# 2025-comprehensive-design/AudioLDM-with-LoRA

Hardware: AMD Instinct MI355X
Metric: unet_denoise_steps_per_sec (higher is better)
Workload: dtype bf16; 1 GPU; audioldm-s-full-v2 UNet + rank-4 LoRA (q,k,v,out), DDIM 200-step schedule, batch 4 x 10 s clips (latent 250x16), CFG 2.5 (UNet batch 8), bf16; per_gpu_batch=4, parallelism=prompt-sharded x1, hip_graph=True, graph_chains=1

## Files before the change

### audioldm_with_lora_amd/csrc/igemm_halo.hip

```cpp
#include "igemm_core.h"
#include "gn_stats.h"

namespace aldm_igemm_detail {

template <int BM, int BN, int WM, int WN, int HP , int S, int EPI , bool GNIN = false>
__global__ __launch_bounds__(512) void igemm_halo_kernel(const IgemmDev p) {
#if defined(__HIP_DEVICE_COMPILE__)
  aldm_touch_kernargs<sizeof(IgemmDev)>();
  static_assert(WM * WN == 8, "8 waves");
  constexpr int NT = 512, RPP = NT / 8;
  constexpr int MI = BM / WM / 16, NI = BN / WN / 16;
  constexpr int W_PASSES = BN / RPP;
  constexpr int D = S - 1;
  constexpr bool STAGGER = false;
  constexpr int HALO_BYTES = HP * RPP * 128;
  constexpr int BSTAGE = BN * 128;
  constexpr unsigned OOB = 0x80000000u;
  static_assert(BN % RPP == 0, "weight tile rows must be whole DMA passes");
  static_assert((D - 1) * W_PASSES + HP < 64, "vmcnt immediate");

  extern __shared__ __attribute__((aligned(16))) char smem[];
  char* const Hs = smem;
  char* const Bring = smem + 2 * HALO_BYTES;
  float* const gtab = reinterpret_cast<float*>(smem + 2 * HALO_BYTES + S * BSTAGE);

  const int tid = threadIdx.x, lane = tid & 63;
  const int wave = __builtin_amdgcn_readfirstlane(tid >> 6);
  const int wm = wave / WN, wn = wave % WN;
  const int W = p.OW, H = p.OH;
  const int HW2 = W + 2;
  const int rows_pt = BM / W;
  const int tpi = (H + rows_pt - 1) / rows_pt;
  int wid = blockIdx.x, split = 0;
  if constexpr (EPI == 3) {
    split = fdiv(wid, p.fd_tiles_m);
    wid -= split * p.tiles_m;
  }
  const int tile_m = fdiv(wid, p.fd_tiles_n), tile_n = wid - tile_m * p.tiles_n;
  const int img = tile_m / tpi, ty0 = (tile_m - img * tpi) * rows_pt;
  const int m0 = img * p.OHW + ty0 * W, n0 = tile_n * BN;
  const int halo_rows = (rows_pt + 2) * HW2;

  const __amdgpu_buffer_rsrc_t rs_x = make_rsrc(p.x, p.x_bytes);
  const __amdgpu_buffer_rsrc_t rs_x2 = make_rsrc(p.x2 ? (const void*)p.x2 : (const void*)p.x, p.x2 ? p.x2_bytes : p.x_bytes);
  const __amdgpu_buffer_rsrc_t rs_w = make_rsrc(p.w, p.w_bytes);

  const int rbase = tid >> 3;
  const int kchunk = (tid & 7) ^ ((rbase >> 1) & 7);
  int h_pix[HP];
  {
    const FastDiv fd_w2 = {p.fd_halo.mul, p.fd_halo.shift};
    const bool up = p.UH > 0;
#pragma unroll
    for (int ps = 0; ps < HP; ++ps) {
      const int hp = rbase + RPP * ps;
      const int hy = fdiv(hp, fd_w2), hx = hp - hy * HW2;
      const int gy = ty0 - 1 + hy, gx = hx - 1;
      const bool ok = hp < halo_rows && (unsigned)gy < (unsigned)H && (unsigned)gx < (unsigned)W;
      const int sy = !up ? gy : (p.UH == 2 * p.IH ? (gy >> 1) : (gy * p.IH) / p.UH);
      const int sx = !up ? gx : (p.UW == 2 * p.IW ? (gx >> 1) : (gx * p.IW) / p.UW);
      h_pix[ps] = ok ? (img * p.IH + sy) * p.IW + sx : -1;
    }
  }
  unsigned b_off[W_PASSES];
#pragma unroll
  for (int ps = 0; ps < W_PASSES; ++ps) {
    const int row = min(n0 + rbase + RPP * ps, p.N - 1);
    b_off[ps] = (unsigned)row * (unsigned)p.Kpad * 2u + kchunk * 16;
  }

  const int nchunks = p.Ctot >> 6;
  const int c_begin = EPI == 3 ? split * (p.kt_per_split / 9) : 0;
  const int c_end = EPI == 3 ? min(nchunks, c_begin + p.kt_per_split / 9) : nchunks;
  const int nitems = (c_end - c_begin) * 9;
  int i_c = c_begin, i_tap = 0;
  auto issue = [&](int item, int stage) {
    const bool live = item < nitems;
    char* bdst = Bring + stage * BSTAGE + wave * 1024;
    if (live && i_tap == 0) {
      const int c0 = i_c << 6;
      const bool src2 = c0 >= p.Cin;
      const int Cs = src2 ? p.Cin2 : p.Cin;
      const int soff = (c0 - (src2 ? p.Cin : 0)) * 2;
      char* hdst = Hs + (i_c & 1) * HALO_BYTES + wave * 1024;
#pragma unroll
      for (int ps = 0; ps < HP; ++ps) {
        const unsigned off = h_pix[ps] >= 0 ? (unsigned)h_pix[ps] * (unsigned)(Cs * 2) + kchunk * 16 : OOB;
        if (src2) __builtin_amdgcn_raw_ptr_buffer_load_lds(rs_x2, (lds_ptr_t)(hdst + ps * (RPP * 128)), 16, off, soff, 0, 0);
        else __builtin_amdgcn_raw_ptr_buffer_load_lds(rs_x, (lds_ptr_t)(hdst + ps * (RPP * 128)), 16, off, soff, 0, 0);
      }
    }
    const int ksoff = live ? (i_tap * p.Ctot + (i_c << 6)) * 2 : 0;
#pragma unroll
    for (int ps = 0; ps < W_PASSES; ++ps)
      __builtin_amdgcn_raw_ptr_buffer_load_lds(rs_w, (lds_ptr_t)(bdst + ps * (RPP * 128)), 16, live ? b_off[ps] : OOB, ksoff, 0, 0);
    if (live) {
      if (++i_tap == 9) { i_tap = 0; ++i_c; }
    }
  };

  f32x4 acc[MI][NI];
#pragma unroll
  for (int i = 0; i < MI; ++i)
#pragma unroll
    for (int j = 0; j < NI; ++j) acc[i][j] = f32x4{0.f, 0.f, 0.f, 0.f};

  const int lrow = lane & 15, lq = lane >> 4;
  int a_hp[MI];
  {
    const FastDiv fd_w = p.fd_ow;
#pragma unroll
    for (int i = 0; i < MI; ++i) {
      const int pl = wm * (BM / WM) + i * 16 + lrow;
      const int ly = fdiv(pl, fd_w), lx = pl - ly * W;
      a_hp[i] = ly * HW2 + lx;
    }
  }

  auto mma_tap = [&](const char* As, const char* Bs, int tap_off) {
#pragma unroll
    for (int ks = 0; ks < 2; ++ks) {
      const int ch = ks * 4 + lq;
      bf16x8 af[MI], wf[NI];
#pragma unroll
      for (int i = 0; i < MI; ++i) {
        const int r = a_hp[i] + tap_off;
        af[i] = *reinterpret_cast<const bf16x8*>(As + r * 128 + swz(r, ch) * 16);
      }
#pragma unroll
      for (int j = 0; j < NI; ++j) {
        const int r = wn * (BN / WN) + j * 16 + lrow;
        wf[j] = *reinterpret_cast<const bf16x8*>(Bs + r * 128 + swz(r, ch) * 16);
      }
#pragma unroll
      for (int i = 0; i < MI; ++i)
#pragma unroll
        for (int j = 0; j < NI; ++j)
          acc[i][j] = __builtin_amdgcn_mfma_f32_16x16x32_bf16(wf[j], af[i], acc[i][j], 0, 0, 0);
    }
  };

#pragma unroll
  for (int s = 0; s < D; ++s) issue(s, s);
  if constexpr (GNIN) {
    const float my_gamma = tid < p.Ctot ? p.gi_gamma[tid] : 0.f, my_beta = tid < p.Ctot ? p.gi_beta[tid] : 0.f;
    const int groups = p.gi_groups, Cg = p.Ctot / groups;
    int lpg = 1;
    while (lpg * 2 * groups <= NT && lpg < 64) lpg *= 2;
    const GnSrc s1{p.x, p.gi_q1, p.Cin, p.gi_bm1, p.gi_tpi1}, s2{p.x2, p.gi_q2, p.Cin2, p.gi_bm2 > 0 ? p.gi_bm2 : 1, p.gi_tpi2};
    const int HWs = p.IH * p.IW;
    const int g = tid / lpg, j = tid - g * lpg;
    float a = 0.f, q2 = 0.f;
    if (g < groups) gn_group_sums(s1, s2, img, HWs, Cg, g, j, lpg, a, q2);
    for (int o = 1; o < lpg; o <<= 1) { a += __shfl_xor(a, o, 64); q2 += __shfl_xor(q2, o, 64); }
    if (g < groups && j == 0) {
      const float n = (float)HWs * (float)Cg;
      const float mu = a / n;
      gtab[1024 + g] = mu;
      gtab[1088 + g] = rsqrtf(fmaxf(q2 / n - mu * mu, 0.f) + p.gi_eps);
    }
    __syncthreads();
    if (tid < p.Ctot) {
      const int gg = tid / Cg;
      const float sc = my_gamma * gtab[1088 + gg];
      gtab[tid] = sc;
      gtab[512 + tid] = my_beta - gtab[1024 + gg] * sc;
    }
    __syncthreads();
  }
  {
    int st = 0, st_fill = D;
    int c_c = c_begin, c_tap = 0, c_dy = 0, c_dx = 0;
    for (int item = 0; item < nitems; ++item) {
      bool halo_young = false;
#pragma unroll
      for (int d = 1; d < D; ++d) {
        const int t = c_tap + d;
        halo_young = halo_young || ((t == 9 || t == 18) && item + d < nitems);
      }
      if (halo_young) wait_vmcnt<(D - 1) * W_PASSES + HP>(); else wait_vmcnt<(D - 1) * W_PASSES>();
      if constexpr (GNIN) {
        if (c_tap == 0) {
          const int cb = (c_c << 6) + kchunk * 8;
          const f32x4 sc0 = *reinterpret_cast<const f32x4*>(gtab + cb), sc1 = *reinterpret_cast<const f32x4*>(gtab + cb + 4);
          const f32x4 sh0 = *reinterpret_cast<const f32x4*>(gtab + 512 + cb), sh1 = *reinterpret_cast<const f32x4*>(gtab + 512 + cb + 4);
          char* hb = Hs + (c_c & 1) * HALO_BYTES + wave * 1024 + lane * 16;
#pragma unroll
          for (int ps = 0; ps < HP; ++ps) {
            if (h_pix[ps] >= 0) {
              const bf16x8 v = *reinterpret_cast<const bf16x8*>(hb + ps * (RPP * 128));
              bf16x8 o;
#pragma unroll
              for (int k = 0; k < 8; ++k) {
                float t = fmaf((float)v[k], k < 4 ? sc0[k & 3] : sc1[k & 3], k < 4 ? sh0[k & 3] : sh1[k & 3]);
                if (p.gi_act == ALDM_ACT_SILU) t = silu_f(t);
                o[k] = (bf16)t;
              }
              *reinterpret_cast<bf16x8*>(hb + ps * (RPP * 128)) = o;
            }
          }
          __builtin_amdgcn_s_waitcnt(0xC07F);
        }
      }
      __builtin_amdgcn_s_barrier();
      if (!(STAGGER && wave >= 4)) issue(item + D, st_fill);
      mma_tap(Hs + (c_c & 1) * HALO_BYTES, Bring + st * BSTAGE, c_dy * HW2 + c_dx);
      if (STAGGER && wave >= 4) issue(item + D, st_fill);
      st = (st + 1 == S) ? 0 : st + 1;
      st_fill = (st_fill + 1 == S) ? 0 : st_fill + 1;
      ++c_tap;
      if (++c_dx == 3) { c_dx = 0; ++c_dy; }
      if (c_tap == 9) { c_tap = 0; c_dy = 0; ++c_c; }
    }
  }
  wait_vmcnt<0>();
  __builtin_amdgcn_s_barrier();

  IgemmDev q = p;
  q.M = min(p.M, min(m0 + BM, (img + 1) * p.OHW));
  q.qtile = tile_m;
  igemm_epilogue<BM, BN, MI, NI, false, NT, EPI>(q, acc, smem, false, m0, n0, wm * (BM / WM), wn * (BN / WN), lrow, lq, split, tid, nullptr);
#endif
}

template <int BM, int BN, int WM, int WN, int HP, int S, int EPI, bool GNIN = false, bool EXT = false>
__global__ __launch_bounds__(768) void igemm_halo_ws_kernel(const IgemmDev p) {
#if defined(__HIP_DEVICE_COMPILE__)
  aldm_touch_kernargs<sizeof(IgemmDev)>();
  static_assert(WM * WN == 8, "8 compute waves");
  constexpr int NTC = 512, NTL = 256, RPP = NTL / 8;
  constexpr int MI = BM / WM / 16, NI = BN / WN / 16;
  constexpr int HPL = HP * 64 / RPP;
  constexpr int W_PASSES = BN / RPP;
  constexpr int D = S - 1;
  constexpr int HALO_BYTES = HP * 64 * 128;
  constexpr int BSTAGE = BN * 128;
  constexpr unsigned OOB = 0x80000000u;
  static_assert((D - 1) * (W_PASSES + HPL) < 64, "vmcnt immediate");
  static_assert(!EXT || (S == 3 && !GNIN), "fused-shortcut form: ring 3, no gnin_*");
  constexpr int NB = EXT ? 3 : 2;

  extern __shared__ __attribute__((aligned(16))) char smem[];
  char* const Hs = smem;
  char* const Bring = smem + NB * HALO_BYTES;
  float* const gtab = reinterpret_cast<float*>(smem + NB * HALO_BYTES + S * BSTAGE);

  const int tid = threadIdx.x, lane = tid & 63;
  const int wave = __builtin_amdgcn_readfirstlane(tid >> 6);
  const bool loader = wave >= NTC / 64;
  const int W = p.OW, H = p.OH;
  const int KWt = p.KW, NTAP = p.KH * p.KW;
  const int HW2 = W + (p.KW - 1) * p.dw;
  const int rows_pt = BM / W;
  const int tpi = (H + rows_pt - 1) / rows_pt;
  int wid = blockIdx.x, split = 0;
  if constexpr (EPI == 3) {
    split = fdiv(wid, p.fd_tiles_m);
    wid -= split * p.tiles_m;
  }
  const int tile_m = fdiv(wid, p.fd_tiles_n), tile_n = wid - tile_m * p.tiles_n;
  const int img = tile_m / tpi, ty0 = (tile_m - img * tpi) * rows_pt;
  const int m0 = img * p.OHW + ty0 * W, n0 = tile_n * BN;
  const int halo_rows = (rows_pt + (p.KH - 1) * p.dh) * HW2;
  const int nchunks = p.Ctot >> 6;
  const int cps = EPI == 3 ? fdiv(p.kt_per_split, p.fd_kw) : 0;
  const int c_begin = EPI == 3 ? split * cps : 0;
  const int c_end = EPI == 3 ? min(nchunks, c_begin + cps) : nchunks;
  const int next = EXT ? (p.C3tot >> 6) : 0;
  const int eps = EPI == 3 ? (next + p.splits - 1) / p.splits : next;
  const int e_begin = EPI == 3 ? min(next, split * eps) : 0;
  const int e_end = min(next, e_begin + eps);
  const int nmain = (c_end - c_begin) * NTAP;
  const int nitems = nmain + (e_end - e_begin);

  if constexpr (GNIN) {
    float my_gamma = 0.f, my_beta = 0.f;
    if (tid < p.Ctot) { my_gamma = p.gi_gamma[tid]; my_beta = p.gi_beta[tid]; }
    const int groups = p.gi_groups, Cg = p.Ctot / groups;
    if (tid < NTC) {
      int lpg = 1;
      while (lpg * 2 * groups <= NTC && lpg < 64) lpg *= 2;
      const GnSrc s1{p.x, p.gi_q1, p.Cin, p.gi_bm1, p.gi_tpi1}, s2{p.x2, p.gi_q2, p.Cin2, p.gi_bm2 > 0 ? p.gi_bm2 : 1, p.gi_tpi2};
      const int HWs = p.IH * p.IW;
      const int g = tid / lpg, j = tid - g * lpg;
      float a = 0.f, q2 = 0.f;
      if (g < groups) gn_group_sums(s1, s2, img, HWs, Cg, g, j, lpg, a, q2);
      for (int o = 1; o < lpg; o <<= 1) { a += __shfl_xor(a, o, 64); q2 += __shfl_xor(q2, o, 64); }
      if (g < groups && j == 0) {
        const float n = (float)HWs * (float)Cg;
        const float mu = a / n;
        gtab[1024 + g] = mu;
        gtab[1088 + g] = rsqrtf(fmaxf(q2 / n - mu * mu, 0.f) + p.gi_eps);
      }
    }
    __syncthreads();
    if (tid < p.Ctot) {
      const int gg = tid / Cg;
      const float sc = my_gamma * gtab[1088 + gg];
      gtab[tid] = sc;
      gtab[512 + tid] = my_beta - gtab[1024 + gg] * sc;
    }
    __syncthreads();
  }

  if (loader) {
    const int lt = tid - NTC, lwave = wave - NTC / 64;
    const __amdgpu_buffer_rsrc_t rs_x = make_rsrc(p.x, p.x_bytes);
    const __amdgpu_buffer_rsrc_t rs_x2 = make_rsrc(p.x2 ? (const void*)p.x2 : (const void*)p.x, p.x2 ? p.x2_bytes : p.x_bytes);
    const __amdgpu_buffer_rsrc_t rs_w = make_rsrc(p.w, p.w_bytes);
    const int rbase = lt >> 3;
    const int kchunk = (lt & 7) ^ ((rbase >> 1) & 7);
    int h_pix[HPL];
    {
      const FastDiv fd_w2 = {p.fd_halo.mul, p.fd_halo.shift};
      const bool up = p.UH > 0;
#pragma unroll
      for (int ps = 0; ps < HPL; ++ps) {
        const int hp = rbase + RPP * ps;
        const int hy = fdiv(hp, fd_w2), hx = hp - hy * HW2;
        const int gy = ty0 - p.ph + hy, gx = hx - p.pw;
        const bool ok = hp < halo_rows && (unsigned)gy < (unsigned)H && (unsigned)gx < (unsigned)W;
      const int sy = !up ? gy : (p.UH == 2 * p.IH ? (gy >> 1) : (gy * p.IH) / p.UH);
      const int sx = !up ? gx : (p.UW == 2 * p.IW ? (gx >> 1) : (gx * p.IW) / p.UW);
        h_pix[ps] = ok ? (img * p.IH + sy) * p.IW + sx : -1;
      }
    }
    unsigned b_off[W_PASSES];
#pragma unroll
    for (int ps = 0; ps < W_PASSES; ++ps) {
      const int row = min(n0 + rbase + RPP * ps, p.N - 1);
      b_off[ps] = (unsigned)row * (unsigned)p.Kpad * 2u + kchunk * 16;
    }
    int i_c = c_begin, i_tap = 0, i_u = 0;
    bool i_ext = EXT && nmain == 0;
    if (i_ext) i_c = e_begin;
    auto issue = [&](int item, int stage) {
      const bool live = item < nitems;
      char* bdst = Bring + stage * BSTAGE + lwave * 1024;
      if (live && i_tap == 0) {
        const int c0 = i_c << 6;
        char* hdst = Hs + (EXT ? i_u % 3 : (i_c & 1)) * HALO_BYTES + lwave * 1024;
        if (EXT && i_ext) {
          const bool s4 = c0 >= p.Cin3;
          const int Cs = s4 ? p.Cin4 : p.Cin3;
          const int soff = (c0 - (s4 ? p.Cin3 : 0)) * 2;
          const __amdgpu_buffer_rsrc_t rs_e = s4 ? make_rsrc(p.x4, p.x4_bytes) : make_rsrc(p.x3, p.x3_bytes);
#pragma unroll
          for (int ps = 0; ps < HPL; ++ps) {
            const unsigned off = h_pix[ps] >= 0 ? (unsigned)h_pix[ps] * (unsigned)(Cs * 2) + kchunk * 16 : OOB;
            __builtin_amdgcn_raw_ptr_buffer_load_lds(rs_e, (lds_ptr_t)(hdst + ps * (RPP * 128)), 16, off, soff, 0, 0);
          }
        } else {
          const bool src2 = c0 >= p.Cin;
          const int Cs = src2 ? p.Cin2 : p.Cin;
          const int soff = (c0 - (src2 ? p.Cin : 0)) * 2;
#pragma unroll
          for (int ps = 0; ps < HPL; ++ps) {
            const unsigned off = h_pix[ps] >= 0 ? (unsigned)h_pix[ps] * (unsigned)(Cs * 2) + kchunk * 16 : OOB;
            if (src2) __builtin_amdgcn_raw_ptr_buffer_load_lds(rs_x2, (lds_ptr_t)(hdst + ps * (RPP * 128)), 16, off, soff, 0, 0);
            else __builtin_amdgcn_raw_ptr_buffer_load_lds(rs_x, (lds_ptr_t)(hdst + ps * (RPP * 128)), 16, off, soff, 0, 0);
          }
        }
      }
      const int ksoff = !live ? 0 : (EXT && i_ext) ? (NTAP * p.Ctot + (i_c << 6)) * 2 : (i_tap * p.Ctot + (i_c << 6)) * 2;
#pragma unroll
      for (int ps = 0; ps < W_PASSES; ++ps)
        __builtin_amdgcn_raw_ptr_buffer_load_lds(rs_w, (lds_ptr_t)(bdst + ps * (RPP * 128)), 16, live ? b_off[ps] : OOB, ksoff, 0, 0);
      if (live) {
        if (EXT && i_ext) { ++i_c; ++i_u; }
        else if (++i_tap == NTAP) {
          i_tap = 0; ++i_c; ++i_u;
          if (EXT && i_c == c_end) { i_ext = true; i_c = e_begin; }
        }
      }
    };
#pragma unroll
    for (int s = 0; s < D; ++s) issue(s, s);
    int st_fill = D;
    int c_c = c_begin, c_tap = 0;
    for (int item = 0; item < nitems; ++item) {
      int young = 0;
#pragma unroll
      for (int d = 1; d < D; ++d) {
        const int t = c_tap + d, it = item + d;
        const bool opens = it < nitems && (it >= nmain || (it < nmain && (t == NTAP || t == 2 * NTAP)));
        young += opens ? 1 : 0;
      }
      if (young == 0) wait_vmcnt<(D - 1) * W_PASSES>();
      else if (young == 1 || D < 3) wait_vmcnt<(D - 1) * W_PASSES + HPL>();
      else wait_vmcnt<(D - 1) * W_PASSES + (D > 2 ? 2 : 1) * HPL>();
      if constexpr (GNIN) {
        if (c_tap == 0) {
          const int cb = (c_c << 6) + kchunk * 8;
          const f32x4 sc0 = *reinterpret_cast<const f32x4*>(gtab + cb), sc1 = *reinterpret_cast<const f32x4*>(gtab + cb + 4);
          const f32x4 sh0 = *reinterpret_cast<const f32x4*>(gtab + 512 + cb), sh1 = *reinterpret_cast<const f32x4*>(gtab + 512 + cb + 4);
          char* hb = Hs + (c_c & 1) * HALO_BYTES + lwave * 1024 + lane * 16;
#pragma unroll
          for (int ps = 0; ps < HPL; ++ps) {
            if (h_pix[ps] >= 0) {
              const bf16x8 v = *reinterpret_cast<const bf16x8*>(hb + ps * (RPP * 128));
              bf16x8 o;
#pragma unroll
              for (int k = 0; k < 8; ++k) {
                float t = fmaf((float)v[k], k < 4 ? sc0[k & 3] : sc1[k & 3], k < 4 ? sh0[k & 3] : sh1[k & 3]);
                if (p.gi_act == ALDM_ACT_SILU) t = silu_f(t);
                o[k] = (bf16)t;
              }
              *reinterpret_cast<bf16x8*>(hb + ps * (RPP * 128)) = o;
            }
          }
          __builtin_amdgcn_s_waitcnt(0xC07F);
        }
      }
      __builtin_amdgcn_s_barrier();
      issue(item + D, st_fill);
      st_fill = (st_fill + 1 == S) ? 0 : st_fill + 1;
      if (item < nmain && ++c_tap == NTAP) { c_tap = 0; ++c_c; }
    }
    wait_vmcnt<0>();
    __builtin_amdgcn_s_barrier();
    return;
  }

  const int wm = wave / WN, wn = wave % WN;
  f32x4 acc[MI][NI];
#pragma unroll
  for (int i = 0; i < MI; ++i)
#pragma unroll
    for (int j = 0; j < NI; ++j) acc[i][j] = f32x4{0.f, 0.f, 0.f, 0.f};
  const int lrow = lane & 15, lq = lane >> 4;
  int a_hp[MI];
#pragma unroll
  for (int i = 0; i < MI; ++i) {
    const int pl = wm * (BM / WM) + i * 16 + lrow;
    const int ly = fdiv(pl, p.fd_ow), lx = pl - ly * W;
    a_hp[i] = ly * HW2 + lx;
  }
  {
    int st = 0, c_c = c_begin, c_tap = 0, c_dy = 0, c_dx = 0, c_u = 0;
    for (int item = 0; item < nitems; ++item) {
      __builtin_amdgcn_s_barrier();
      const bool seg = EXT && item >= nmain;
      const char* As = Hs + (EXT ? c_u % 3 : (c_c & 1)) * HALO_BYTES;
      const char* Bs = Bring + st * BSTAGE;
      const int tap_off = seg ? HW2 + 1 : c_dy * p.dh * HW2 + c_dx * p.dw;
#pragma unroll
      for (int ks = 0; ks < 2; ++ks) {
        const int ch = ks * 4 + lq;
        bf16x8 af[MI], wf[NI];
#pragma unroll
        for (int i = 0; i < MI; ++i) {
          const int r = a_hp[i] + tap_off;
          af[i] = *reinterpret_cast<const bf16x8*>(As + r * 128 + swz(r, ch) * 16);
        }
#pragma unroll
        for (int j = 0; j < NI; ++j) {
          const int r = wn * (BN / WN) + j * 16 + lrow;
          wf[j] = *reinterpret_cast<const bf16x8*>(Bs + r * 128 + swz(r, ch) * 16);
        }
#pragma unroll
        for (int i = 0; i < MI; ++i)
#pragma unroll
          for (int j = 0; j < NI; ++j) acc[i][j] = __builtin_amdgcn_mfma_f32_16x16x32_bf16(wf[j], af[i], acc[i][j], 0, 0, 0);
      }
      st = (st + 1 == S) ? 0 : st + 1;
      if (seg) { ++c_u; continue; }
      ++c_tap;
      if (++c_dx == KWt) { c_dx = 0; ++c_dy; }
      if (c_tap == NTAP) { c_tap = 0; c_dy = 0; ++c_c; ++c_u; }
    }
  }
  __builtin_amdgcn_s_waitcnt(0xC07F);
  __builtin_amdgcn_s_barrier();
  IgemmDev q = p;
  q.M = min(p.M, min(m0 + BM, (img + 1) * p.OHW));
  q.qtile = tile_m;
  igemm_epilogue<BM, BN, MI, NI, false, NTC, EPI>(q, acc, smem, false, m0, n0, wm * (BM / WM), wn * (BN / WN), lrow, lq, split, tid, nullptr);
#endif
}

template <int BM, int BN, int WM, int WN, int HP, int S, int EPI, bool GNIN = false, bool WS = false, bool EXT = false>
int launch_halo_v(const IgemmDev& d, hipStream_t st) {
  static_assert(!EXT || WS, "the fused-shortcut form exists for the wave-specialised kernel only");
  constexpr size_t lds_loop = (EXT ? 3 : 2) * (size_t)HP * 64 * 128 + (size_t)S * BN * 128 + (GNIN ? (1024 + 128) * sizeof(float) : 0);
  constexpr size_t lds = lds_loop > (size_t)EpiCfg<BM, BN>::BYTES ? lds_loop : (size_t)EpiCfg<BM, BN>::BYTES;
  static_assert(lds <= 160 * 1024, "LDS budget");
  static unsigned long long attr_done = 0;
  void (*kern)(const IgemmDev);
  if constexpr (EXT) kern = igemm_halo_ws_kernel<BM, BN, WM, WN, HP, S, EPI, false, true>;
  else if constexpr (WS) kern = igemm_halo_ws_kernel<BM, BN, WM, WN, HP, S, EPI, GNIN>;
  else kern = igemm_halo_kernel<BM, BN, WM, WN, HP, S, EPI, GNIN>;
  if (int rc = aldm_set_max_lds(reinterpret_cast<const void*>(kern), (int)lds, &attr_done, "igemm_halo")) return rc;
  const int rows_pt = BM / d.OW;
  const int need = WS ? (rows_pt + (d.KH - 1) * d.dh) * (d.OW + (d.KW - 1) * d.dw) : (rows_pt + 2) * (d.OW + 2);
  if (BM % d.OW != 0 || need > HP * 64) {
    aldm_set_error("igemm_halo: image width %d / filter %dx%d does not fit the %dx%d halo tile (%d halo rows of %d)", d.OW, d.KH, d.KW, BM, BN, need, HP * 64);
    return ALDM_E_UNSUPPORTED;
  }
  IgemmDev dd = d;
  if (WS) dd.fd_kw = make_fastdiv((unsigned)(d.KH * d.KW));
  dd.tiles_n = cdiv(d.N, BN);
  dd.fd_tiles_n = make_fastdiv((unsigned)dd.tiles_n);
  dd.fd_halo = make_fastdiv((unsigned)(WS ? d.OW + (d.KW - 1) * d.dw : d.OW + 2));
  const int tpi = cdiv(d.OH, rows_pt);
  dd.tiles_m = d.B * tpi * dd.tiles_n;
  dd.fd_tiles_m = make_fastdiv((unsigned)dd.tiles_m);
  dim3 grid(d.B * tpi * dd.tiles_n * (EPI == 3 ? d.splits : 1), 1, 1);
  hipLaunchKernelGGL(kern, grid, dim3(WS ? 768 : 512), lds, st, dd);
  return aldm_launch_status("igemm_halo");
}

template <int BM, int BN, int WM, int WN, int HP, int S>
int launch_halo_ext(const IgemmDev& d, hipStream_t st) {
  if (d.gi_gamma) {
    aldm_set_error("igemm_halo: gnin_* launches take no second-source segment");
    return ALDM_E_UNSUPPORTED;
  }
  if (d.splits > 1) return launch_halo_v<BM, BN, WM, WN, HP, S, 3, false, true, true>(d, st);
  if (d.out_act == ALDM_ACT_NONE && d.post_act == ALDM_ACT_NONE)
    return d.qstat ? launch_halo_v<BM, BN, WM, WN, HP, S, 4, false, true, true>(d, st) : launch_halo_v<BM, BN, WM, WN, HP, S, 1, false, true, true>(d, st);
  return launch_halo_v<BM, BN, WM, WN, HP, S, 0, false, true, true>(d, st);
}

template <int BM, int BN, int WM, int WN, int HP, int S, bool WS = false>
int launch_halo(const IgemmDev& d, hipStream_t st) {
  if (d.splits > 1) {
    if (d.gi_gamma) {
      aldm_set_error("igemm_halo: gnin_* launches are not split");
      return ALDM_E_UNSUPPORTED;
    }
    return launch_halo_v<BM, BN, WM, WN, HP, S, 3, false, WS>(d, st);
  }
  if (d.gi_gamma) {
    if (d.out_act != ALDM_ACT_NONE || d.post_act != ALDM_ACT_NONE) {
      aldm_set_error("igemm_halo: gnin_* launches take no output activation");
      return ALDM_E_UNSUPPORTED;
    }
    return d.qstat ? launch_halo_v<BM, BN, WM, WN, HP, S, 4, true, WS>(d, st) : launch_halo_v<BM, BN, WM, WN, HP, S, 1, true, WS>(d, st);
  }
  if (d.out_act == ALDM_ACT_NONE && d.post_act == ALDM_ACT_NONE)
    return d.qstat ? launch_halo_v<BM, BN, WM, WN, HP, S, 4, false, WS>(d, st) : launch_halo_v<BM, BN, WM, WN, HP, S, 1, false, WS>(d, st);
  return launch_halo_v<BM, BN, WM, WN, HP, S, 0, false, WS>(d, st);
}

}

int aldm_launch_halo(const aldm_igemm_detail::IgemmDev& d0, int tile, int ring, hipStream_t st) {
  using namespace aldm_igemm_detail;
  IgemmDev d = d0;
  const bool ws = tile == ALDM_TILE_HALO_128x128_WS || tile == ALDM_TILE_HALO_64x128_WS;
  if (ws && d.KH == 1 && d.OH == 1 && d.IH == 1 && d.UH == 0 && d.ph == 0 && d.dh == 1 && d.sh == 1 && d.C3tot == 0 && !d.gi_gamma) {
    d.KH = d.KW; d.KW = 1; d.dh = d.dw; d.dw = 1; d.ph = d.pw; d.pw = 0;
    d.OH = d.OW; d.OW = 1; d.IH = d.IW; d.IW = 1; d.sh = d.sw; d.sw = 1;
    d.fd_ow = make_fastdiv(1u);
    d.fd_ohw = make_fastdiv((unsigned)d.OHW);
  }
  const bool same = ws ? (d.KH % 2 == 1 && d.KW % 2 == 1 && 2 * d.ph == (d.KH - 1) * d.dh && 2 * d.pw == (d.KW - 1) * d.dw &&
                          ((d.KH == 3 && d.KW == 3 && d.dh == 1 && d.dw == 1) || (d.C3tot == 0 && !d.gi_gamma && d.UH == 0)))
                       : (d.KH == 3 && d.KW == 3 && d.ph == 1 && d.pw == 1 && d.dh == 1 && d.dw == 1);
  const bool ok = same && d.sh == 1 && d.sw == 1 &&
                  d.in_act == ALDM_ACT_NONE && d.Cin % 64 == 0 && d.Cin2 % 64 == 0 && d.dilate == 0 &&
                  !d.ln_s && !d.geglu && d.x_bytes < 0x80000000u && d.x2_bytes < 0x80000000u &&
                  ((d.UH == 0 && d.UW == 0) || (d.UH > 0 && d.UW > 0)) && d.OH == (d.UH ? d.UH : d.IH) && d.OW == (d.UW ? d.UW : d.IW);
  if (!ok) {
    aldm_set_error("igemm_halo: needs a stride-1 'same' convolution on the LDS-DMA path (Cin %% 64 == 0, no gather activation): 3x3, or -- wave-specialised tiles -- any odd filter with dilation");
    return ALDM_E_UNSUPPORTED;
  }
  if (d.C3tot > 0) {
    const bool fits = d.UH == 0 && d.C3tot % 64 == 0 && d.Cin3 % 64 == 0 && d.x3_bytes < 0x80000000u && d.x4_bytes < 0x80000000u;
    if (fits && tile == ALDM_TILE_HALO_128x128_WS && (128 / d.OW + 2) * (d.OW + 2) <= 192) return launch_halo_ext<128, 128, 4, 2, 3, 3>(d, st);
    if (fits && tile == ALDM_TILE_HALO_64x128_WS) return launch_halo_ext<64, 128, 2, 4, 2, 3>(d, st);
    aldm_set_error("igemm_halo: the second-source segment needs a wave-specialised halo tile whose halo fits three DMA passes (OW >= 8 at 128 rows)");
    return ALDM_E_UNSUPPORTED;
  }
  if (tile == ALDM_TILE_HALO_128x128_WS) {
    if ((128 / d.OW + (d.KH - 1) * d.dh) * (d.OW + (d.KW - 1) * d.dw) > 192) {
      if (ring == 4) return launch_halo<128, 128, 4, 2, 5, 4, true>(d, st);
      return launch_halo<128, 128, 4, 2, 5, 3, true>(d, st);
    }
    if (ring == 4) return launch_halo<128, 128, 4, 2, 3, 4, true>(d, st);
    return launch_halo<128, 128, 4, 2, 3, 3, true>(d, st);
  }
  if (tile == ALDM_TILE_HALO_64x128_WS) {
    if (ring == 4) return launch_halo<64, 128, 2, 4, 2, 4, true>(d, st);
    return launch_halo<64, 128, 2, 4, 2, 3, true>(d, st);
  }
  if (tile == ALDM_TILE_HALO_128x128) {
    if ((128 / d.OW + 2) * (d.OW + 2) > 192) {
      if (ring == 2) return launch_halo<128, 128, 4, 2, 5, 2>(d, st);
      if (ring == 4) return launch_halo<128, 128, 4, 2, 5, 4>(d, st);
      return launch_halo<128, 128, 4, 2, 5, 3>(d, st);
    }
    if (ring == 2) return launch_halo<128, 128, 4, 2, 3, 2>(d, st);
    if (ring == 4) return launch_halo<128, 128, 4, 2, 3, 4>(d, st);
    return launch_halo<128, 128, 4, 2, 3, 3>(d, st);
  }
  if (ring == 2) return launch_halo<64, 128, 2, 4, 2, 2>(d, st);
  if (ring == 4) return launch_halo<64, 128, 2, 4, 2, 4>(d, st);
  return launch_halo<64, 128, 2, 4, 2, 3>(d, st);
}
```

Baseline: 356.9 denoise_steps/s.

## Overlap GroupNorm stats with ring prefill and share halo normalisation across waves

For the wave-specialised GroupNorm-fused conv kernel, two new forms are added and both are on by default through environment switches. Ring-first lets the loader waves issue the initial weight and halo DMA before the compute waves finish the GroupNorm statistics and tables, so the stats prologue overlaps the first loads. Shared normalisation spreads the in-LDS normalise+SiLU of each halo chunk across all 768 threads, with extra barriers, instead of leaving it to the loader waves alone. The cost is added barrier synchronisation per channel chunk and more template instantiations.

```diff
diff --git a/audioldm_with_lora_amd/csrc/igemm_halo.hip b/audioldm_with_lora_amd/csrc/igemm_halo.hip
--- a/audioldm_with_lora_amd/csrc/igemm_halo.hip
+++ b/audioldm_with_lora_amd/csrc/igemm_halo.hip
@@ -1,3 +1,5 @@
+#include <cstdlib>
+
 #include "igemm_core.h"
 #include "gn_stats.h"
 
@@ -223,7 +225,7 @@
 #endif
 }
 
-template <int BM, int BN, int WM, int WN, int HP, int S, int EPI, bool GNIN = false, bool EXT = false>
+template <int BM, int BN, int WM, int WN, int HP, int S, int EPI, bool GNIN = false, bool EXT = false, bool RF = false, bool SH = false>
 __global__ __launch_bounds__(768) void igemm_halo_ws_kernel(const IgemmDev p) {
 #if defined(__HIP_DEVICE_COMPILE__)
   aldm_touch_kernargs<sizeof(IgemmDev)>();
@@ -238,6 +240,10 @@
   constexpr unsigned OOB = 0x80000000u;
   static_assert((D - 1) * (W_PASSES + HPL) < 64, "vmcnt immediate");
   static_assert(!EXT || (S == 3 && !GNIN), "fused-shortcut form: ring 3, no gnin_*");
+  static_assert(GNIN || (!RF && !SH), "ring-first / shared normalisation are forms of the gnin_* launches");
+  constexpr int NT = NTC + NTL;
+  constexpr int NPP = (HP * 512 + NT - 1) / NT;
+  static_assert(((NT / 8) >> 1) % 8 == 0, "a thread's pieces share one XOR term, hence one channel base");
   constexpr int NB = EXT ? 3 : 2;
 
   extern __shared__ __attribute__((aligned(16))) char smem[];
@@ -273,7 +279,7 @@
   const int nmain = (c_end - c_begin) * NTAP;
   const int nitems = nmain + (e_end - e_begin);
 
-  if constexpr (GNIN) {
+  auto gn_tables = [&]() __attribute__((always_inline)) {
     float my_gamma = 0.f, my_beta = 0.f;
     if (tid < p.Ctot) { my_gamma = p.gi_gamma[tid]; my_beta = p.gi_beta[tid]; }
     const int groups = p.gi_groups, Cg = p.Ctot / groups;
@@ -301,7 +307,50 @@
       gtab[512 + tid] = my_beta - gtab[1024 + gg] * sc;
     }
     __syncthreads();
-  }
+  };
+  if constexpr (GNIN && !RF) gn_tables();
+
+  int sh_cb = 0;
+  unsigned sh_ok = 0;
+  auto sh_setup = [&]() __attribute__((always_inline)) {
+    const FastDiv fd_w2 = {p.fd_halo.mul, p.fd_halo.shift};
+    const int r0 = tid >> 3;
+    sh_cb = ((tid & 7) ^ ((r0 >> 1) & 7)) * 8;
+#pragma unroll
+    for (int k = 0; k < NPP; ++k) {
+      const int hp = r0 + (NT / 8) * k;
+      const int hy = fdiv(hp, fd_w2), hx = hp - hy * HW2;
+      const int gy = ty0 - p.ph + hy, gx = hx - p.pw;
+      const bool ok = hp < HP * 64 && hp < halo_rows && (unsigned)gy < (unsigned)H && (unsigned)gx < (unsigned)W;
+      sh_ok |= ok ? 1u << k : 0u;
+    }
+  };
+  auto sh_norm = [&](int c) __attribute__((always_inline)) {
+    if (sh_ok) {
+      const int cb = (c << 6) + sh_cb;
+      const f32x4 sc0 = *reinterpret_cast<const f32x4*>(gtab + cb), sc1 = *reinterpret_cast<const f32x4*>(gtab + cb + 4);
+      const f32x4 sh0 = *reinterpret_cast<const f32x4*>(gtab + 512 + cb), sh1 = *reinterpret_cast<const f32x4*>(gtab + 512 + cb + 4);
+      char* hb = Hs + (c & 1) * HALO_BYTES + tid * 16;
+      bf16x8 v[NPP];
+#pragma unroll
+      for (int k = 0; k < NPP; ++k)
+        if ((k + 1) * NT <= HP * 512 || tid + k * NT < HP * 512) v[k] = *reinterpret_cast<const bf16x8*>(hb + k * (NT * 16));
+#pragma unroll
+      for (int k = 0; k < NPP; ++k) {
+        if ((sh_ok >> k) & 1u) {
+          bf16x8 o;
+#pragma unroll
+          for (int e = 0; e < 8; ++e) {
+            float t = fmaf((float)v[k][e], e < 4 ? sc0[e & 3] : sc1[e & 3], e < 4 ? sh0[e & 3] : sh1[e & 3]);
+            if (p.gi_act == ALDM_ACT_SILU) t = silu_f(t);
+            o[e] = (bf16)t;
+          }
+          *reinterpret_cast<bf16x8*>(hb + k * (NT * 16)) = o;
+        }
+      }
+    }
+    __builtin_amdgcn_s_waitcnt(0xC07F);
+  };
 
   if (loader) {
     const int lt = tid - NTC, lwave = wave - NTC / 64;
@@ -376,6 +425,11 @@
     };
 #pragma unroll
     for (int s = 0; s < D; ++s) issue(s, s);
+    if constexpr (SH) sh_setup();
+    if constexpr (RF) {
+      __builtin_amdgcn_s_barrier();
+      __builtin_amdgcn_s_barrier();
+    }
     int st_fill = D;
     int c_c = c_begin, c_tap = 0;
     for (int item = 0; item < nitems; ++item) {
@@ -389,7 +443,21 @@
       if (young == 0) wait_vmcnt<(D - 1) * W_PASSES>();
       else if (young == 1 || D < 3) wait_vmcnt<(D - 1) * W_PASSES + HPL>();
       else wait_vmcnt<(D - 1) * W_PASSES + (D > 2 ? 2 : 1) * HPL>();
-      if constexpr (GNIN) {
+      if constexpr (SH) {
+        if (c_tap == 0) {
+          __builtin_amdgcn_s_barrier();
+          issue(item + D, st_fill);
+          sh_norm(c_c);
+          __builtin_amdgcn_s_barrier();
+        } else {
+          __builtin_amdgcn_s_barrier();
+          issue(item + D, st_fill);
+        }
+        st_fill = (st_fill + 1 == S) ? 0 : st_fill + 1;
+        if (item < nmain && ++c_tap == NTAP) { c_tap = 0; ++c_c; }
+        continue;
+      }
+      if constexpr (GNIN && !SH) {
         if (c_tap == 0) {
           const int cb = (c_c << 6) + kchunk * 8;
           const f32x4 sc0 = *reinterpret_cast<const f32x4*>(gtab + cb), sc1 = *reinterpret_cast<const f32x4*>(gtab + cb + 4);
@@ -422,6 +490,8 @@
     return;
   }
 
+  if constexpr (SH) sh_setup();
+  if constexpr (RF) gn_tables();
   const int wm = wave / WN, wn = wave % WN;
   f32x4 acc[MI][NI];
 #pragma unroll
@@ -439,6 +509,13 @@
   {
     int st = 0, c_c = c_begin, c_tap = 0, c_dy = 0, c_dx = 0, c_u = 0;
     for (int item = 0; item < nitems; ++item) {
+      if constexpr (SH) {
+        if (c_tap == 0) {
+          __builtin_amdgcn_s_waitcnt(0xC07F);
+          __builtin_amdgcn_s_barrier();
+          sh_norm(c_c);
+        }
+      }
       __builtin_amdgcn_s_barrier();
       const bool seg = EXT && item >= nmain;
       const char* As = Hs + (EXT ? c_u % 3 : (c_c & 1)) * HALO_BYTES;
@@ -479,16 +556,17 @@
 #endif
 }
 
-template <int BM, int BN, int WM, int WN, int HP, int S, int EPI, bool GNIN = false, bool WS = false, bool EXT = false>
+template <int BM, int BN, int WM, int WN, int HP, int S, int EPI, bool GNIN = false, bool WS = false, bool EXT = false, bool RF = false, bool SH = false>
 int launch_halo_v(const IgemmDev& d, hipStream_t st) {
   static_assert(!EXT || WS, "the fused-shortcut form exists for the wave-specialised kernel only");
+  static_assert((GNIN && WS) || (!RF && !SH), "ring-first / shared normalisation: wave-specialised gnin_* launches only");
   constexpr size_t lds_loop = (EXT ? 3 : 2) * (size_t)HP * 64 * 128 + (size_t)S * BN * 128 + (GNIN ? (1024 + 128) * sizeof(float) : 0);
   constexpr size_t lds = lds_loop > (size_t)EpiCfg<BM, BN>::BYTES ? lds_loop : (size_t)EpiCfg<BM, BN>::BYTES;
   static_assert(lds <= 160 * 1024, "LDS budget");
   static unsigned long long attr_done = 0;
   void (*kern)(const IgemmDev);
   if constexpr (EXT) kern = igemm_halo_ws_kernel<BM, BN, WM, WN, HP, S, EPI, false, true>;
-  else if constexpr (WS) kern = igemm_halo_ws_kernel<BM, BN, WM, WN, HP, S, EPI, GNIN>;
+  else if constexpr (WS) kern = igemm_halo_ws_kernel<BM, BN, WM, WN, HP, S, EPI, GNIN, false, RF, SH>;
   else kern = igemm_halo_kernel<BM, BN, WM, WN, HP, S, EPI, GNIN>;
   if (int rc = aldm_set_max_lds(reinterpret_cast<const void*>(kern), (int)lds, &attr_done, "igemm_halo")) return rc;
   const int rows_pt = BM / d.OW;
@@ -522,6 +600,12 @@
   return launch_halo_v<BM, BN, WM, WN, HP, S, 0, false, true, true>(d, st);
 }
 
+inline int gnin_form() {
+  const char* rf = getenv("ALDM_GNIN_RING_FIRST");
+  const char* sh = getenv("ALDM_GNIN_SHARED");
+  return ((rf && atoi(rf) == 0) ? 0 : 1) | ((sh && atoi(sh) == 0) ? 0 : 2);
+}
+
 template <int BM, int BN, int WM, int WN, int HP, int S, bool WS = false>
 int launch_halo(const IgemmDev& d, hipStream_t st) {
   if (d.splits > 1) {
@@ -535,6 +619,17 @@
     if (d.out_act != ALDM_ACT_NONE || d.post_act != ALDM_ACT_NONE) {
       aldm_set_error("igemm_halo: gnin_* launches take no output activation");
       return ALDM_E_UNSUPPORTED;
+    }
+    if constexpr (WS) {
+      const int form = gnin_form();
+#define ALDM_GNIN_FORM(RFV, SHV)                                                                          \
+  return d.qstat ? launch_halo_v<BM, BN, WM, WN, HP, S, 4, true, true, false, RFV, SHV>(d, st)            \
+                 : launch_halo_v<BM, BN, WM, WN, HP, S, 1, true, true, false, RFV, SHV>(d, st)
+      if (form == 3) ALDM_GNIN_FORM(true, true);
+      if (form == 2) ALDM_GNIN_FORM(false, true);
+      if (form == 1) ALDM_GNIN_FORM(true, false);
+      ALDM_GNIN_FORM(false, false);
+#undef ALDM_GNIN_FORM
     }
     return d.qstat ? launch_halo_v<BM, BN, WM, WN, HP, S, 4, true, WS>(d, st) : launch_halo_v<BM, BN, WM, WN, HP, S, 1, true, WS>(d, st);
   }
```

Measured after the change: 359.0 denoise_steps/s, median of 6. Within noise of the previous version (+0.6%).
